# Tung-I/Dual-awareness-Attention-for-Few-shot-Object-Detection

Measured on AMD Instinct MI355X. Metric: query-images/sec (res50, way=2, shot=3, bs=4 per GPU, train-mode forward), higher is better.
Workload: dtype f32 (operands, accumulation, results; multiplies as an exact bf16x3 split, six bf16 MFMA products each)

## Files before the change

### dual-awareness-attention-for-few-shot-object-detection_amd/csrc/igemm.hip

```cpp
#include "common.h"
#include "../../include/dana_hip_debug.h"
#include <stdlib.h>
#include <atomic>

namespace {

typedef float f32x16 __attribute__((ext_vector_type(16)));
typedef unsigned int u32x4 __attribute__((ext_vector_type(4)));

struct IgemmParams {
  const float* A;
  const float* Bw;
  float* C;
  const float* scale;
  const float* shift;
  const float* residual;
  const float* mask;
  long ldm;
  int M, N, K;
  int IH, IW, OH, OW, Cin, KH, KW, stride, pad;
  int M0, IH1, IW1, OH1, OW1, pix1;
  float* C1;
  const float* residual1;
  long ldc1, ldr1;
// ... 6 lines not shown
  int vec_io;
  int vec_ss;
  int tiles_m, tiles_n;
  const float* A2;
  int lda2, IH2, IW2, stride2, K1;
  int IH21, IW21, pix21;
  int bpre;
  const void* Bw2;
  const float* scale2;
  const float* shift2;
  int N2, relu2;
  unsigned a2_bytes;
  int apre, a_rows;
  int res_sample, res_h, res_w, res_oh, res_ow;
  unsigned res_bytes;
  unsigned long long* trace;
};

constexpr int BK = 32;
constexpr int LDS_LD = 36;
constexpr unsigned OOB = 0x80000000u;

__device__ __forceinline__ int xcd_remap(int bid, int nwg) {
  const int q = nwg / 8, r = nwg % 8;
  const int xcd = bid % 8, local = bid / 8;
  return (xcd < r ? xcd * (q + 1) : r * (q + 1) + (xcd - r) * q) + local;
}

__device__ __forceinline__ float4 ldg_b128(__amdgpu_buffer_rsrc_t r, unsigned off) {
  u32x4 v = __builtin_amdgcn_raw_buffer_load_b128(r, (int)off, 0, 0);
// ... 391 lines not shown
#pragma unroll
        for (int r = 0; r < 16; ++r) {
          const int m = m0 + wm * (BM / 2) + i * 32 + (r & 3) + 8 * (r >> 2) + 4 * lh;
          if (m < p.M && ncol[j] < p.N) {
            const bool s1 = m >= p.M0;
            float v = acc[i][j][r] * scv[j] + shv[j];
            if (p.residual) v += s1 ? p.residual1[(long)(m - p.M0) * p.ldr1 + ncol[j]] : p.residual[(long)m * p.ldr + ncol[j]];
            if (p.relu) v = fmaxf(v, 0.f);
            if (p.mask && !(p.mask[(long)m * p.ldm + ncol[j]] > 0.f)) v = 0.f;
            (s1 ? p.C1 + (long)(m - p.M0) * p.ldc1 : Cb + (long)m * p.ldc)[ncol[j]] = v;
          }
        }
  }
}

template <int BM, int BN, int STEM, int BPRE = 0, int FUSE = 0, int ELDS = 0, int RSMP = 0>
__device__ __forceinline__ void igemm_split_body(const IgemmParams& p) {
  static_assert(!RSMP || (!STEM && !FUSE && !ELDS), "sampled residual: register epilogue of the plain conv / GEMM forms");
  constexpr int TM = BM / 64, TN = BN / 64;
  constexpr int RA = BM / 64;
  constexpr int RB = BPRE ? (3 * BN * 2 + 255) / 256 : BN / 64;
  constexpr int CLD = BN + 4;
  extern __shared__ __attribute__((aligned(16))) float smem[];
  unsigned* As = (unsigned*)smem;
  unsigned* Bs = As + 2 * 3 * BM * SLD;

  const int tid = threadIdx.x;
  const int lane = tid & 63, wave = tid >> 6;
  const int wm = wave >> 1, wn = wave & 1;
  const int li = lane & 31, lh = lane >> 5;

  const unsigned long long t_start = p.trace ? __builtin_readcyclecounter() : 0ull;
  const unsigned long long w_start = p.trace ? wall_clock64() : 0ull;
// ... 182 lines not shown
  auto read_frags = [&](int buf, u32x4(&fa)[3][TM], u32x4(&fb)[3][TN]) {
    const unsigned* as = As + buf * 3 * BM * SLD + (wm * (BM / 2) + li) * SLD + rcol;
    const unsigned* bs = Bs + buf * 3 * BN * SLD + (wn * (BN / 2) + li) * SLD + rcol;
#pragma unroll
    for (int pc = 0; pc < 3; ++pc) {
#pragma unroll
      for (int i = 0; i < TM; ++i) fa[pc][i] = *(const u32x4*)(as + (pc * BM + i * 32) * SLD);
#pragma unroll
      for (int j = 0; j < TN; ++j) fb[pc][j] = *(const u32x4*)(bs + (pc * BN + j * 32) * SLD);
    }
  };

  load_tile(ra0, rb0);
  load_tile(ra1, rb1);
  __builtin_amdgcn_sched_barrier(0);
#pragma unroll
  for (int i = 0; i < TM; ++i)
#pragma unroll
    for (int j = 0; j < TN; ++j)
#pragma unroll
      for (int r = 0; r < 16; ++r) acc[i][j][r] = 0.f;
#pragma unroll
  for (int i = 0; i < TM; ++i)
#pragma unroll
    for (int j = 0; j < TN; ++j) asm volatile("" : "+a"(acc[i][j]));
  __builtin_amdgcn_sched_barrier(0);
  store_tile(0, ra0, rb0);
  __syncthreads();
  load_tile(ra0, rb0);
  read_frags(0, fa0, fb0);
  store_tile(1, ra1, rb1);
  __syncthreads();

  auto k_step = [&](int t, const u32x4(&fa)[3][TM], const u32x4(&fb)[3][TN], u32x4(&na)[3][TM], u32x4(&nb)[3][TN],
                    const float4(&cv_a)[RA], const float4(&cv_b)[RB], float4(&ld_a)[RA], float4(&ld_b)[RB]) {
    const int bw_ = t & 1, br_ = bw_ ^ 1;
// ... 422 lines not shown
    }
  }
  if (p.trace && tid == 0) {
    unsigned long long* tr = p.trace + ((long)blockIdx.z * gridDim.x + blockIdx.x) * 8;
    tr[0] = t_start;
    tr[1] = t_loop;
    tr[2] = t_loop_end;
    tr[3] = __builtin_readcyclecounter();
    tr[4] = (unsigned long long)__builtin_amdgcn_s_getreg((31 << 11) | 4) | ((unsigned long long)__builtin_amdgcn_s_getreg((31 << 11) | 20) << 32);
    tr[5] = wall_clock64();
    tr[6] = w_start;
    tr[7] = 0;
  }
}

template <int BM, int BN, int STEM, int BPRE = 0, int FUSE = 0, int ELDS = 0, int RSMP = 0>
__global__ void __launch_bounds__(256, 2) igemm_split_kernel(IgemmParams p) {
  igemm_split_body<BM, BN, STEM, BPRE, FUSE, ELDS, RSMP>(p);
}
template <int STEM, int BPRE, int ELDS, int RSMP = 0>
__global__ void __launch_bounds__(256, 1) __attribute__((amdgpu_num_vgpr(192))) igemm_split_kernel_128(IgemmParams p) {
  igemm_split_body<128, 128, STEM, BPRE, 0, ELDS, RSMP>(p);
}

template <int BN, int NST, int APRE, int DF = 0>
__global__ void __launch_bounds__(256, NST == 2 ? 3 : (NST == 3 ? 2 : 1)) igemm_dma_kernel(IgemmParams p) {
  static_assert(APRE || NST == 2, "fp32 activation rows: two stages");
  static_assert(!DF || (APRE && NST >= 3), "two fragment sets: planes x planes, three or more stages");
  constexpr int BM = 128, TM = 2, TN = BN / 64;
  constexpr int STAGE_B = 3 * (BM + BN) * 32;
  constexpr int NPB = 3 * BN / 32, PB = (NPB + 3) / 4;
  constexpr int NDMA = (APRE ? 3 : 0) + PB;
  constexpr int AHEAD = NST == 2 ? 2 : NST - 1;
  constexpr int RA = BM / 64;
  extern __shared__ __attribute__((aligned(16))) float smem[];
  const int tid = threadIdx.x;
  const int lane = tid & 63, wave = __builtin_amdgcn_readfirstlane(tid >> 6);
// ... 341 lines not shown
  uint2 h, m, l;
  split3(v, h, m, l);
  const int ks = k4 / SBK, kk = k4 - ks * SBK;
  unsigned short* o = out + blockIdx.y * 3 * (long)n * kp + (((long)ks * 3) * n + row) * SBK + kk;
  *(uint2*)o = h;
  *(uint2*)(o + (long)n * SBK) = m;
  *(uint2*)(o + 2 * (long)n * SBK) = l;
}

std::atomic<int>& epilogue_mode_cell() {
  static std::atomic<int> cell(0);
  return cell;
}

std::atomic<int> g_last_form(0);
constexpr int form_code(int family, int bm, int bn, int stem, int bpre, int fuse, int elds, int nst, int apre, int df) {
  return family | (bm / 64) << 4 | (bn / 64) << 6 | stem << 8 | bpre << 9 | fuse << 10 | elds << 11 | nst << 12 | apre << 16 | df << 17;
}

template <int BM, int BN, int STEM>
int launch(const IgemmParams& p0, int batch, hipStream_t s) {
  g_last_form.store(form_code(DANA_IGEMM_FAMILY_F32, BM, BN, STEM, 0, 0, 0, 0, 0, 0), std::memory_order_relaxed);
  IgemmParams p = p0;
  p.tiles_m = (p.M + BM - 1) / BM;
  p.tiles_n = (p.N + BN - 1) / BN;
  size_t lds = (size_t)2 * (BM + BN) * LDS_LD * sizeof(float);
  const size_t lds_c = (size_t)BM * (BN + 4) * sizeof(float);
  if (lds_c > lds) lds = lds_c;
  static DeviceOnce attr;
  attr.once([&] { return hipFuncSetAttribute((const void*)igemm_f32_kernel<BM, BN, STEM>, hipFuncAttributeMaxDynamicSharedMemorySize, (int)lds); });
  dim3 grid(p.tiles_m * p.tiles_n, 1, batch);
  igemm_f32_kernel<BM, BN, STEM><<<grid, 256, lds, s>>>(p);
  return 0;
}

template <int BM, int BN, int STEM = 0, int BPRE = 0, int FUSE = 0, int ELDS = 0, int RSMP = 0>
int launch_split(const IgemmParams& p0, int batch, hipStream_t s) {
  if constexpr (BPRE == 0 && FUSE == 0) {
    if (p0.bpre) return launch_split<BM, BN, STEM, 1, 0, ELDS, RSMP>(p0, batch, s);
  }
  if constexpr (ELDS == 0 && FUSE == 0 && RSMP == 0) {
    if (epilogue_mode_cell().load(std::memory_order_relaxed)) return launch_split<BM, BN, STEM, BPRE, 0, 1>(p0, batch, s);
  }
  g_last_form.store(form_code(BM * BN >= 128 * 128 ? DANA_IGEMM_FAMILY_SPLIT_128 : DANA_IGEMM_FAMILY_SPLIT, BM, BN, STEM, BPRE, FUSE ? 1 : 0,
                              ELDS, 0, 0, 0), std::memory_order_relaxed);
  IgemmParams p = p0;
  p.tiles_m = (p.M + BM - 1) / BM;
  p.tiles_n = (p.N + BN - 1) / BN;
  size_t lds = (size_t)2 * 3 * (BM + BN) * SLD * sizeof(unsigned);
  const size_t lds_c = (size_t)BM * (BN + 4) * sizeof(float);
  if (lds_c > lds && ELDS) lds = lds_c;
  if (FUSE && lds < (size_t)4 * 3 * BM * 16 * 2) lds = (size_t)4 * 3 * BM * 16 * 2;
  if (FUSE == 2 || RSMP) lds += (size_t)BM * 4;
  dim3 grid(p.tiles_m * p.tiles_n, 1, batch);
  static DeviceOnce attr;
  if constexpr (BM * BN >= 128 * 128) {
    attr.once([&] { return hipFuncSetAttribute((const void*)igemm_split_kernel_128<STEM, BPRE, ELDS, RSMP>, hipFuncAttributeMaxDynamicSharedMemorySize,
                                (int)lds); });
    igemm_split_kernel_128<STEM, BPRE, ELDS, RSMP><<<grid, 256, lds, s>>>(p);
  } else {
    attr.once([&] { return hipFuncSetAttribute((const void*)igemm_split_kernel<BM, BN, STEM, BPRE, FUSE, ELDS, RSMP>,
                                hipFuncAttributeMaxDynamicSharedMemorySize, (int)lds); });
    igemm_split_kernel<BM, BN, STEM, BPRE, FUSE, ELDS, RSMP><<<grid, 256, lds, s>>>(p);
  }
  return 0;
}

template <int BN, int NST, int APRE, int DF = 0>
int launch_dma(const IgemmParams& p0, int batch, hipStream_t s) {
  g_last_form.store(form_code(DANA_IGEMM_FAMILY_DMA, 128, BN, 0, 1, 0, 0, NST, APRE, DF), std::memory_order_relaxed);
  IgemmParams p = p0;
  p.tiles_m = (p.M + 127) / 128;
  p.tiles_n = (p.N + BN - 1) / BN;
  const size_t lds = (size_t)NST * 3 * (128 + BN) * 32;
  static DeviceOnce attr;
  attr.once([&] { return hipFuncSetAttribute((const void*)igemm_dma_kernel<BN, NST, APRE, DF>, hipFuncAttributeMaxDynamicSharedMemorySize, (int)lds); });
  dim3 grid(p.tiles_m * p.tiles_n, 1, batch);
  igemm_dma_kernel<BN, NST, APRE, DF><<<grid, 256, lds, s>>>(p);
// ... 31 lines not shown
}
unsigned long long* g_trace = nullptr;

int dispatch_sampled(const IgemmParams& p, int batch, hipStream_t s) {
  const int mode = mfma_mode_cell().load(std::memory_order_relaxed);
  if (!mode || p.apre || p.mask || p.KH * p.KW > 32 || p.M0 != p.M || epilogue_mode_cell().load(std::memory_order_relaxed)) return -1;
  if (p.N <= 64) return -1;
  if (mode == 3) return launch_split<64, 64, 0, 0, 0, 0, 1>(p, batch, s);
  if (mode == 4) return launch_split<128, 128, 0, 0, 0, 0, 1>(p, batch, s);
  if (p.N <= 256 && p.N % 128 != 0 && p.N % 128 <= 32) return launch_split<64, 64, 0, 0, 0, 0, 1>(p, batch, s);
  const long t128 = (long)((p.M + 127) / 128) * ((p.N + 127) / 128) * batch;
  if (t128 < 100) return launch_split<64, 64, 0, 0, 0, 0, 1>(p, batch, s);
  return launch_split<128, 128, 0, 0, 0, 0, 1>(p, batch, s);
}

int dispatch(const IgemmParams& p, int batch, int stem, hipStream_t s) {
  if (p.res_sample) return stem ? -1 : dispatch_sampled(p, batch, s);
  if (stem) {
    const int smode = mfma_mode_cell().load(std::memory_order_relaxed);
    return smode ? launch_split<128, 64, 1>(p, batch, s) : launch<128, 64, 1>(p, batch, s);
  }
  const int mode = mfma_mode_cell().load(std::memory_order_relaxed);
  if (p.apre) {
    const int pp_env = pp_stages_cell().load(std::memory_order_relaxed);
    const long t128 = (long)((p.M + 127) / 128) * ((p.N + 127) / 128) * batch;
    const int stages = pp_env >= 0 ? pp_env : ((t128 < 400 || p.K >= 1024) ? 13 : 2);
    if (p.N <= 64) return stages == 2 ? launch_dma<64, 2, 1>(p, batch, s) : launch_dma<64, 3, 1>(p, batch, s);
    if (stages == 2) return launch_dma<128, 2, 1>(p, batch, s);
    if (stages == 4) return launch_dma<128, 4, 1>(p, batch, s);
    if (stages == 6) return launch_dma<128, 6, 1>(p, batch, s);
    if (stages == 13) return launch_dma<128, 3, 1, 1>(p, batch, s);
// ... 430 lines not shown
                 long batch_a, long batch_b, long batch_c, float alpha, int flags, dana_stream_t stream) {
  DANA_CHECK_ARG(m >= 0 && n >= 0 && k > 0 && batch >= 0, "dana_gemm_nt: bad shape m=%d n=%d k=%d", m, n, k);
  if (m == 0 || n == 0 || batch == 0) return DANA_OK;
  DANA_CHECK_ARG(a && b && c, "dana_gemm_nt: null pointer");
  DANA_CHECK_ARG(k % 4 == 0 && lda % 4 == 0 && ldb % 4 == 0 && batch_a % 4 == 0 && batch_b % 4 == 0,
                 "dana_gemm_nt: k, lda, ldb and batch strides must be multiples of 4 (16-byte rows)");
  const int bpre = (flags & DANA_W_SPLIT3) ? 1 : 0;
  DANA_CHECK_ARG(!bpre || (dana_get_mfma_mode() != 0 && ldb % SBK == 0 && ldb >= k && batch_b % 8 == 0 && n > 8),
                 "dana_gemm_nt: DANA_W_SPLIT3 needs the split kernel, ldb = k rounded up to 16, n > 8");
  const int apre = (flags & DANA_A_SPLIT3) ? 1 : 0;
  DANA_CHECK_ARG(!apre || (bpre && lda % SBK == 0 && lda >= k && batch_a % 8 == 0),
                 "dana_gemm_nt: DANA_A_SPLIT3 needs DANA_W_SPLIT3 too, lda = k rounded up to 16");
  DANA_CHECK_ARG(lda >= k && ldb >= k && ldc >= n, "dana_gemm_nt: leading dimension smaller than the row");
  DANA_CHECK_ARG(((uintptr_t)a & 15) == 0 && ((uintptr_t)b & 15) == 0, "dana_gemm_nt: a/b must be 16-byte aligned");
  DANA_CHECK_ARG(!residual || batch == 1, "dana_gemm_nt: residual only with batch == 1");
  hipStream_t s = (hipStream_t)stream;
  if (n <= 8 && batch == 1 && !residual) {
    gemm_skinny_kernel<8><<<dana_ceil_div(m, 4), 256, 0, s>>>(a, b, c, scale, shift, m, n, k, lda, ldb, ldc, alpha,
                                                              (flags & DANA_EPI_RELU) ? 1 : 0);
    DANA_CHECK_LAUNCH("dana_gemm_nt(skinny)");
    return DANA_OK;
  }
  const long a_bytes = apre ? (long)3 * m * lda * 2 : ((long)(m - 1) * lda + k) * 4;
  const long b_bytes = bpre ? (long)3 * n * ldb * 2 : ((long)(n - 1) * ldb + k) * 4;
  DANA_CHECK_ARG(a_bytes < (long)OOB && b_bytes < (long)OOB, "dana_gemm_nt: operand slice >= 2 GiB; split it");
  IgemmParams p;
  memset(&p, 0, sizeof(p));
  p.A = a;
  p.Bw = b;
  p.C = c;
// ... 13 lines not shown
  p.pad = 0;
  p.lda = (int)lda;
  p.ldb = (int)ldb;
  p.a_bytes = (unsigned)a_bytes;
  p.b_bytes = (unsigned)b_bytes;
  p.ldc = ldc;
  p.ldr = ldr > 0 ? ldr : ldc;
  p.batch_a = apre ? batch_a / 2 : batch_a;
  p.batch_b = bpre ? batch_b / 2 : batch_b;
  p.apre = apre;
  p.a_rows = m;
  p.batch_c = batch_c;
  p.bpre = bpre;
  p.alpha = alpha;
  p.relu = (flags & DANA_EPI_RELU) ? 1 : 0;
  run(p, batch, 0, s);
  DANA_CHECK_LAUNCH("dana_gemm_nt");
  return DANA_OK;
}

}
```

### dual-awareness-attention-for-few-shot-object-detection_amd/csrc/winograd.hip

```cpp
#include "common.h"
#include "../../include/dana_hip.h"

namespace {

typedef unsigned int u32x4 __attribute__((ext_vector_type(4)));
constexpr unsigned OOB = 0x80000000u;

__device__ __forceinline__ float4 f4add(float4 a, float4 b) { return make_float4(a.x + b.x, a.y + b.y, a.z + b.z, a.w + b.w); }
__device__ __forceinline__ float4 f4sub(float4 a, float4 b) { return make_float4(a.x - b.x, a.y - b.y, a.z - b.z, a.w - b.w); }

__global__ void __launch_bounds__(256)
wino_filter_kernel(const float* __restrict__ w, float* __restrict__ U, int cout, int cin) {
  const long i = (long)blockIdx.x * blockDim.x + threadIdx.x;
  if (i >= (long)cout * cin) return;
  const int ci = (int)(i % cin);
  const long co = i / cin;
  float g[3][3];
#pragma unroll
  for (int r = 0; r < 3; ++r)
#pragma unroll
    for (int c = 0; c < 3; ++c) g[r][c] = w[((co * 3 + r) * 3 + c) * cin + ci];
  float t[4][3];
#pragma unroll
  for (int c = 0; c < 3; ++c) {
// ... 572 lines not shown
    wino4_output_kernel<<<dana_ceil_div(p.tiles * N4, 256), 256, 0, s>>>(M, output, scale, shift, mask_act, ldm, h, w, N4,
                                                                        p.th, p.tw, p.tiles, ldc,
                                                                        (flags & DANA_EPI_RELU) ? 1 : 0, 0, 0, res, ldr, res_group);
  DANA_CHECK_LAUNCH("dana_conv3x3_winograd4_nhwc(output transform)");
  return DANA_OK;
}

int dana_conv3x3_winograd4_nhwc_masked(const float* input, const float* u, float* output, const float* scale,
                                       const float* shift, const float* mask_act, int batch, int h, int w, int cin,
                                       int cout, long in_pix_stride, long out_pix_stride, long mask_pix_stride,
                                       int flags, void* workspace, size_t workspace_bytes, dana_stream_t stream) {
  return wino4_impl(input, u, output, scale, shift, mask_act, nullptr, 0, 1, batch, h, w, cin, cout, in_pix_stride,
                    out_pix_stride, mask_pix_stride, flags, workspace, workspace_bytes, stream);
}

int dana_conv3x3_winograd4_nhwc_sub(const float* input, const float* u, float* output, const float* scale,
                                    const float* shift, int batch, int h, int w, int cin, int cout, long in_pix_stride,
                                    long out_pix_stride, int sub, int flags, void* workspace, size_t workspace_bytes,
                                    dana_stream_t stream) {
  return wino4_impl(input, u, output, scale, shift, nullptr, nullptr, 0, 1, batch, h, w, cin, cout, in_pix_stride,
                    out_pix_stride, 0, flags, workspace, workspace_bytes, stream, sub);
}

size_t dana_conv3x3_winograd4_dual_workspace_bytes(int n0, int h0, int w0, int n1, int h1, int w1, int cin, int cout) {
  if (n0 < 0 || n1 < 0 || cin <= 0 || cout <= 0) return 0;
  const long t0 = n0 > 0 ? wino_plan(n0, h0, w0, cin, cout, 4).tiles : 0, t1 = n1 > 0 ? wino_plan(n1, h1, w1, cin, cout, 4).tiles : 0;
  return dana_align_up((size_t)36 * (t0 + t1) * cin * 4, 256) + dana_align_up((size_t)36 * (t0 + t1) * cout * 4, 256);
}

int dana_conv3x3_winograd4_nhwc_dual(const float* input, const float* u, float* out0, float* out1, const float* scale,
// ... 75 lines not shown
```

### dual-awareness-attention-for-few-shot-object-detection_amd/dana.py

```python
import contextlib
import math
import time
from types import SimpleNamespace

import numpy as np
import torch
import torch.nn as nn
import torch.nn.functional as F

from . import ops
from .config import cfg
from . import targets as T
from .cached_inputs import (BankEpisode, ClassSweep, QueryBank, QueryBatch, SupportBank, SupportCache,
                            check_cached_forward, query_batch_size, query_device, read_inputs, resolve_bank_episode,
                            resolve_query_batch, resolve_shot_views)


class Bottleneck(nn.Module):
    expansion = 4

    def __init__(self, inplanes, planes, stride=1, downsample=None):
        super().__init__()
        self.conv1 = nn.Conv2d(inplanes, planes, kernel_size=1, stride=stride, bias=False)
        self.bn1 = nn.BatchNorm2d(planes)
# ... 123 lines not shown
        self.unary_gamma = 0.1
        self.semantic_enhance = semantic_enhance
        self.rpn_reduce_dim = rpn_reduce_dim
        self.rcnn_reduce_dim = rcnn_reduce_dim
        self.pos_encoding = pos_encoding
        self.pool_feat_dim = 1024
        self.rcnn_dim = 64
        self.use_winograd = True
        self.winograd_tile = 4
        self.winograd_min_cin = 128
        self.presplit_weights = True
        self.merge_trunk = False
        self.merge_from = 0
        self.fold_roi_pe = True
        self.fold_roi_attn = True
        self.prefetch_dgrad = "layer4"
        self.rpn_side_role = "wgrad"
        self.nms_inclusive = False
        dim_in = self.pool_feat_dim

        def lin(i, o):
            m = nn.Linear(i, o)
            nn.init.normal_(m.weight, std=0.01)
            nn.init.constant_(m.bias, 0)
            return m

        self.rpn_unary_layer = lin(dim_in, 1)
        self.rcnn_unary_layer = lin(dim_in, 1)
        self.rpn_adapt_q_layer = lin(dim_in, rpn_reduce_dim)
        self.rpn_adapt_k_layer = lin(dim_in, rpn_reduce_dim)
# ... 1050 lines not shown
        return corr, (fh, fw), dict(feat=sfeat, map=(sh_, sw_), kp=kp, unary=unary, s_t=s_t, rpn_done=rpn_done)

    def _rpn_attention(self, f, corr, fh, fw, sup):
        B, Cs, NP, dev, main = f.B, f.Cs, f.NP, f.dev, f.main
        d = self.rpn_reduce_dim
        hw = fh * fw
        L = sup["map"][0] * sup["map"][1]
        K1 = f.shot * L
        kp, unary, s_t = sup["kp"], sup["unary"], sup["s_t"]
        scale, seg_w = self._attn_scale(f)
        _, bq = self._w(self.rpn_adapt_q_layer)
        qb3, qld = self._lin_b(self.rpn_adapt_q_layer)
        qp = ops.gemm_nt(corr, qb3, B * hw, d, 1024, lda=2048, ldb=qld, shift=bq)
        ops.colmean_sub_(qp, B, hw, d)
        f.mark("rpn-level Q projection")
        if sup["rpn_done"] is not None:
            main.wait_event(sup["rpn_done"])
        f.mark("... wait for the support side (trunk + RPN-level K / unary / S^T chain)")
        att = None
        if f.sweep is not None:
            scores = torch.empty((B, hw, Cs * K1), dtype=torch.float32, device=dev)
            ops.gemm_nt(qp, kp, hw, Cs * K1, d, out=scores, ldc=Cs * K1, batch=B, batch_a=hw * d, batch_b=Cs * K1 * d,
                        batch_c=hw * Cs * K1, alpha=1.0 / math.sqrt(d))
            a_p = torch.empty((NP, hw, K1), dtype=torch.float32, device=dev)
            if seg_w is not None:
                ops.attn_softmax_unary_sweep_w(scores, a_p, unary, B, Cs, hw, f.shot, L, K1, K1, K1, self.unary_gamma, seg_w)
            else:
                ops.attn_softmax_unary_sweep(scores, a_p, unary, B, Cs, hw, f.shot, L, K1, K1, K1, self.unary_gamma, scale)
            if f.maps is not None:
                f.maps["rpn_w"] = a_p
# ... 21 lines not shown
        if f.inter is not None:
            f.inter["corr"] = (corr, B, fh, fw)
        if f.ctx is not None:
            f.ctx.update(corr=corr, fh=fh, fw=fw, qp=qp, scores=scores)
        f.mark("rpn-level attention (incl. wait for support stream)")
        return att

    @staticmethod
    def _attn_scale(f):
        if f.maps is None:
            return 1.0 / f.shot, f.seg_w
        if f.seg_w is not None and "slot_w" not in f.maps:
            f.maps["slot_w"] = (f.seg_w > 0).to(torch.float32)
        return 1.0, f.maps.get("slot_w")

    def _rpn_conv_stage(self, f, corr, att, fh, fw):
        if f.sweep is not None:
            return self._rpn_conv_sweep(f.plan, corr, att, f.B, f.Cs, fh, fw, f.product)
        kv = [] if f.ctx is not None else None
        x = self._rpn_conv(f.plan, corr.view(-1)[1024:] if f.product else corr, f.B, fh, fw, in_stride=2048, keep_v=kv)
        if kv:
            f.ctx["rpn_v"] = kv[0]
        return x

    def _roi_support(self, f, sup):
        ctx = f.ctx
        if f.cache is None:
            proposals_start = ops.record_event()
            with ops.on_stream(f.sup_stream):
                f.sup_stream.wait_event(proposals_start)
                sh_, sw_ = sup["map"]
                Ns = f.B * f.way * f.shot
                if f.episode is not None:
# ... 210 lines not shown
```

### dual-awareness-attention-for-few-shot-object-detection_amd/ops.py

```python
import collections
import contextlib
import ctypes
import time as _time

import torch

from ._lib import lib, DanaError

HOST_WAIT = [0.0]

NCHW, NHWC = 0, 1
EPI_RELU, CONV_STEM7, W_SPLIT3, A_SPLIT3 = 1, 2, 256, 512

PROFILE = None
PROF_ROLE = None


def _prof_begin():
    if PROFILE is None:
        return None
    e = torch.cuda.Event(enable_timing=True)
    e.record()
    return e


def _prof_end(e0, tag, flops, nbytes=0.0, executed=None):
    if e0 is not None:
# ... 756 lines not shown
    elif sub != 1:
        lib().call("dana_conv3x3_winograd4_nhwc_sub", _p(x), up, _p(out), _p(scale), _p(shift), batch, h, w, cin, cout,
                   in_stride, out_stride, int(sub), (EPI_RELU if relu else 0) | wfl, _p(ws), ws.numel(), _stream())
    else:
        lib().call("dana_conv3x3_winograd%s_nhwc_masked" % sfx, _p(x), up, _p(out), _p(scale), _p(shift), _p(mask), batch,
                   h, w, cin, cout, in_stride, out_stride, mask_stride, (EPI_RELU if relu else 0) | wfl, _p(ws), ws.numel(),
                   _stream())
    if keep_v is not None and m == 4:
        keep_v.append(ws)
    _prof_end(e0, ("wino3x3 M=%d N=%d K=%d s1", (batch * h * w, cout, 9 * cin)), 2.0 * batch * h * w * cout * 9 * cin,
              4.0 * (m + 2) * (m + 2) * (batch * ((h + m - 1) // m) * ((w + m - 1) // m) * (cin + cout) + cout * cin),
              executed=2.0 * (m + 2) * (m + 2) * batch * ((h + m - 1) // m) * ((w + m - 1) // m) * cin * cout)
    return out, oh, ow


def set_mfma_mode(mode):
    prev = lib().query("dana_get_mfma_mode")
    lib().call("dana_set_mfma_mode", int(mode))
    return prev


def get_mfma_mode():
    return lib().query("dana_get_mfma_mode")


def force_tile(tile):
    lib().call("dana_debug_force_tile", int(tile))


def cumask_stream(cus_per_xcd, n_xcd=8, cus_in_xcd=32):
# ... 28 lines not shown

def get_dma_kernel():
    return lib().query("dana_debug_get_dma_kernel")


def set_pp_stages(v):
    prev = lib().query("dana_debug_get_pp_stages")
    lib().call("dana_debug_set_pp_stages", int(v))
    return prev


def get_pp_stages():
    return lib().query("dana_debug_get_pp_stages")


IgemmForm = collections.namedtuple("IgemmForm", "family bm bn stem bpre fuse elds nst apre df")
_IGEMM_FAMILIES = {0: None, 1: "f32", 2: "split", 3: "split_128", 4: "dma"}


def decode_igemm_form(code):
    return IgemmForm(_IGEMM_FAMILIES[code & 15], (code >> 4 & 3) * 64, (code >> 6 & 3) * 64, code >> 8 & 1, code >> 9 & 1,
                     code >> 10 & 1, code >> 11 & 1, code >> 12 & 15, code >> 16 & 1, code >> 17 & 1)


def last_igemm_form():
    return decode_igemm_form(lib().query("dana_debug_last_igemm_form"))


@contextlib.contextmanager
def igemm_forms(tile=0, dma=-1, pp=-1, epilogue=0):
    prev_dma, prev_pp, prev_epi = get_dma_kernel(), get_pp_stages(), lib().query("dana_get_epilogue_mode")
    try:
        if tile:
            force_tile(tile)
        set_dma_kernel(dma)
        set_pp_stages(pp)
        set_epilogue_mode(epilogue)
# ... 11 lines not shown

def _splitk_slices(m, n, k, batch):
    if batch != 1 or n % 4 or n <= 8 or k < 512 or k % 16:
        return 1
    tiles = ((m + 63) // 64) * ((n + 63) // 64)
    if tiles >= 512:
        return 1
    s = max(1, min(8, round(768.0 / tiles)))
    steps = k // 16
    while s > 1 and (steps % s or k // s < 256):
        s -= 1
    return s


def gemm_nt(a, b, m, n, k, lda=0, ldb=0, out=None, ldc=0, scale=None, shift=None, residual=None, ldr=0, batch=1,
            batch_a=0, batch_b=0, batch_c=0, alpha=1.0, relu=False, k_true=0, force_slices=0):
    bp, wfl = _wf(b)
    if isinstance(a, W3):
        if not wfl or a.n != m or a.k != k or batch != a.batch:
            raise ValueError("gemm_nt: split activation planes need split weights and matching m / k / batch")
        out = torch.empty((batch, m, n) if batch > 1 else (m, n), dtype=torch.float32, device=a.t.device) if out is None else out
        ldc = ldc or n
        e0 = _prof_begin()
        lib().call("dana_gemm_nt", _p(a.t), bp, _p(out), _p(scale), _p(shift), _p(residual), m, n, k, a.kp, b.kp, ldc,
                   ldr, batch, 3 * m * a.kp, 3 * n * b.kp, batch_c or m * n, float(alpha), (EPI_RELU if relu else 0) | wfl | A_SPLIT3,
                   _stream())
        _prof_end(e0, ("gemm M=%d N=%d K=%d b%d", (m, n, k, batch)), 2.0 * batch * m * n * (k_true or k),
                  batch * (6.0 * (m * k + n * k) + 4.0 * m * n * (2 if residual is not None else 1)))
        return out
    _chk(a, "a")
    lda = lda or k
    if wfl:
        if ldb not in (0, k) or batch != 1 or b.n != n or b.k != k:
            raise ValueError("gemm_nt: a split weight is used whole ([n][k] as split)")
        ldb = b.kp
    else:
        ldb = ldb or k
    if out is None:
        out = torch.empty((batch, m, n) if batch > 1 else (m, n), dtype=torch.float32, device=a.device)
        ldc = n
        batch_c = m * n
    e0 = _prof_begin()
    slices = (force_slices or _splitk_slices(m, n, k, batch)) if SPLIT_K else 1
    if wfl and slices > 1 and (k // slices) % 16:
        slices = 1
    if slices > 1:
        kc = k // slices
        part = torch.empty((slices, m, n), dtype=torch.float32, device=a.device)
        lib().call("dana_gemm_nt", _p(a), bp, _p(part), None, None, None, m, n, kc, lda, ldb, n, 0, slices, kc,
                   kc * 3 * n if wfl else kc, m * n, 1.0, wfl, _stream())
        lib().call("dana_splitk_reduce", _p(part), slices, m, n, _p(out), ldc, _p(scale), _p(shift), _p(residual), ldr,
                   float(alpha), EPI_RELU if relu else 0, _stream())
    else:
        lib().call("dana_gemm_nt", _p(a), bp, _p(out), _p(scale), _p(shift), _p(residual), m, n, k, lda, ldb, ldc,
                   ldr, batch, batch_a, batch_b, batch_c, float(alpha), (EPI_RELU if relu else 0) | wfl, _stream())
    _prof_end(e0, ("gemm M=%d N=%d K=%d b%d", (m, n, k, batch)), 2.0 * batch * m * n * (k_true or k),
              4.0 * batch * (m * k + n * k + m * n * (2 if residual is not None else 1)))
    return out


def nchw_to_nhwc(x, cpad=None, out=None, out_stride=0):
    x = _chk(x.contiguous(), "x")
    B, C, H, W = x.shape
    cpad = cpad or C
    if out is None:
        out = torch.empty((B, H, W, cpad), dtype=torch.float32, device=x.device)
    lib().call("dana_nchw_to_nhwc", _p(x), _p(out), B, C, H, W, cpad, out_stride, _stream())
    return out


def nhwc_to_nchw(x, B, C, H, W, in_stride=0):
    _chk(x, "x")
# ... 706 lines not shown
```

### include/dana_hip.h

```cpp
#ifndef DANA_HIP_H
#define DANA_HIP_H
#include <stddef.h>
#include <stdint.h>

#ifdef __cplusplus
extern "C" {
#endif

typedef void* dana_stream_t;

#define DANA_LAYOUT_NCHW 0
#define DANA_LAYOUT_NHWC 1

#define DANA_EPI_RELU 1
#define DANA_CONV_STEM7 2
#define DANA_W_SPLIT3 256
#define DANA_A_SPLIT3 512

const char* dana_last_error(void);
int dana_abi_version(void);

int dana_set_mfma_mode(int mode);
int dana_get_mfma_mode(void);


int dana_roi_align_forward(const float* input, const float* rois, float* output, int batch, int channels,
                           int height, int width, int num_rois, float spatial_scale, int pooled_h,
                           int pooled_w, int sampling_ratio, int layout, long in_pix_stride,
                           long out_pix_stride, float* output2, const float* add2, long out2_pix_stride,
                           dana_stream_t stream);

int dana_roi_align_backward(const float* grad_out, const float* rois, float* grad_in, int batch, int channels,
// ... 128 lines not shown
int dana_conv3x3_winograd_nhwc_masked(const float* input, const float* u, float* output, const float* scale,
                                      const float* shift, const float* mask_act, int batch, int h, int w, int cin,
                                      int cout, long in_pix_stride, long out_pix_stride, long mask_pix_stride,
                                      int flags, void* workspace, size_t workspace_bytes, dana_stream_t stream);

int dana_winograd4_filter_transform(const float* w_packed, float* u, int cout, int cin, dana_stream_t stream);
size_t dana_conv3x3_winograd4_workspace_bytes(int batch, int h, int w, int cin, int cout);
int dana_conv3x3_winograd4_nhwc_masked(const float* input, const float* u, float* output, const float* scale,
                                       const float* shift, const float* mask_act, int batch, int h, int w, int cin,
                                       int cout, long in_pix_stride, long out_pix_stride, long mask_pix_stride,
                                       int flags, void* workspace, size_t workspace_bytes, dana_stream_t stream);
int dana_conv3x3_winograd4_nhwc_sub(const float* input, const float* u, float* output, const float* scale,
                                    const float* shift, int batch, int h, int w, int cin, int cout, long in_pix_stride,
                                    long out_pix_stride, int sub, int flags, void* workspace, size_t workspace_bytes,
                                    dana_stream_t stream);
int dana_conv3x3_winograd_nhwc_grouped_res(const float* input, const float* u, float* output, const float* scale,
                                           const float* shift, const float* residual, int batch, int h, int w, int cin,
                                           int cout, long in_pix_stride, long out_pix_stride, long res_pix_stride,
                                           int res_group, int tile, int flags, void* workspace, size_t workspace_bytes,
                                           dana_stream_t stream);
size_t dana_conv3x3_winograd4_dual_workspace_bytes(int n0, int h0, int w0, int n1, int h1, int w1, int cin, int cout);
int dana_conv3x3_winograd4_nhwc_dual(const float* input, const float* u, float* out0, float* out1, const float* scale,
                                     const float* shift, int n0, int h0, int w0, int n1, int h1, int w1, int cin,
                                     int cout, long in_pix_stride, long out0_pix_stride, long out1_pix_stride, int flags,
                                     void* workspace, size_t workspace_bytes, dana_stream_t stream);
int dana_conv3x3_winograd4_nhwc_dual_masked(const float* input, const float* u, float* out0, float* out1,
                                            const float* scale, const float* shift, const float* mask0,
                                            const float* mask1, int n0, int h0, int w0, int n1, int h1, int w1, int cin,
                                            int cout, long in_pix_stride, long out0_pix_stride, long out1_pix_stride,
                                            long mask0_pix_stride, long mask1_pix_stride, int flags, void* workspace,
// ... 296 lines not shown
```

Baseline: 731.7.

## Start RPN 3x3 conv on first half of channels before waiting on support side

Adds a channel-range-partitioned Winograd F(4x4,3x3) conv whose GEMM can seed its accumulators from the existing output, so a conv can be split into two K-halves. The first half of the RPN conv (channels 0-1024 of the query-only correlation input) is launched before the main stream waits on the support-side event, and the second half plus the output transform runs afterwards. This moves work off the critical path behind the cross-stream wait. In exchange the seeded GEMM rereads and rewrites the M workspace, paying one extra input-transform launch and extra memory traffic.

```diff
diff --git a/dual-awareness-attention-for-few-shot-object-detection_amd/csrc/igemm.hip b/dual-awareness-attention-for-few-shot-object-detection_amd/csrc/igemm.hip
--- a/dual-awareness-attention-for-few-shot-object-detection_amd/csrc/igemm.hip
+++ b/dual-awareness-attention-for-few-shot-object-detection_amd/csrc/igemm.hip
@@ -44,6 +44,7 @@
   int apre, a_rows;
   int res_sample, res_h, res_w, res_oh, res_ow;
   unsigned res_bytes;
+  int seed;
   unsigned long long* trace;
 };
 
@@ -465,9 +466,10 @@
   }
 }
 
-template <int BM, int BN, int STEM, int BPRE = 0, int FUSE = 0, int ELDS = 0, int RSMP = 0>
+template <int BM, int BN, int STEM, int BPRE = 0, int FUSE = 0, int ELDS = 0, int RSMP = 0, int SEED = 0>
 __device__ __forceinline__ void igemm_split_body(const IgemmParams& p) {
   static_assert(!RSMP || (!STEM && !FUSE && !ELDS), "sampled residual: register epilogue of the plain conv / GEMM forms");
+  static_assert(!SEED || (!STEM && !FUSE && !ELDS && !RSMP), "seeded accumulators: register epilogue of the plain GEMM forms");
   constexpr int TM = BM / 64, TN = BN / 64;
   constexpr int RA = BM / 64;
   constexpr int RB = BPRE ? (3 * BN * 2 + 255) / 256 : BN / 64;
@@ -680,12 +682,31 @@
   load_tile(ra0, rb0);
   load_tile(ra1, rb1);
   __builtin_amdgcn_sched_barrier(0);
-#pragma unroll
-  for (int i = 0; i < TM; ++i)
-#pragma unroll
-    for (int j = 0; j < TN; ++j)
-#pragma unroll
-      for (int r = 0; r < 16; ++r) acc[i][j][r] = 0.f;
+  if constexpr (SEED) {
+    const int rows_valid = (p.M - m0) < BM ? (p.M - m0) : BM;
+    const int ldc4 = (int)p.ldc * 4;
+    const __amdgpu_buffer_rsrc_t rc_seed =
+        __builtin_amdgcn_make_buffer_rsrc((void*)(Cb + (long)m0 * p.ldc), 0, rows_valid * ldc4, 0x00020000);
+    const int lrow = wm * (BM / 2) + 4 * lh;
+#pragma unroll
+    for (int j = 0; j < TN; ++j) {
+      const int ncol = n0 + wn * (BN / 2) + j * 32 + li;
+      const unsigned vo = ncol < p.N ? (unsigned)(lrow * ldc4 + ncol * 4) : OOB;
+#pragma unroll
+      for (int i = 0; i < TM; ++i)
+#pragma unroll
+        for (int r = 0; r < 16; ++r)
+          acc[i][j][r] = __builtin_bit_cast(
+              float, __builtin_amdgcn_raw_buffer_load_b32(rc_seed, (int)(vo + (unsigned)((i * 32 + (r & 3) + 8 * (r >> 2)) * ldc4)), 0, 0));
+    }
+  } else {
+#pragma unroll
+    for (int i = 0; i < TM; ++i)
+#pragma unroll
+      for (int j = 0; j < TN; ++j)
+#pragma unroll
+        for (int r = 0; r < 16; ++r) acc[i][j][r] = 0.f;
+  }
 #pragma unroll
   for (int i = 0; i < TM; ++i)
 #pragma unroll
@@ -1138,13 +1159,13 @@
   }
 }
 
-template <int BM, int BN, int STEM, int BPRE = 0, int FUSE = 0, int ELDS = 0, int RSMP = 0>
+template <int BM, int BN, int STEM, int BPRE = 0, int FUSE = 0, int ELDS = 0, int RSMP = 0, int SEED = 0>
 __global__ void __launch_bounds__(256, 2) igemm_split_kernel(IgemmParams p) {
-  igemm_split_body<BM, BN, STEM, BPRE, FUSE, ELDS, RSMP>(p);
-}
-template <int STEM, int BPRE, int ELDS, int RSMP = 0>
+  igemm_split_body<BM, BN, STEM, BPRE, FUSE, ELDS, RSMP, SEED>(p);
+}
+template <int STEM, int BPRE, int ELDS, int RSMP = 0, int SEED = 0>
 __global__ void __launch_bounds__(256, 1) __attribute__((amdgpu_num_vgpr(192))) igemm_split_kernel_128(IgemmParams p) {
-  igemm_split_body<128, 128, STEM, BPRE, 0, ELDS, RSMP>(p);
+  igemm_split_body<128, 128, STEM, BPRE, 0, ELDS, RSMP, SEED>(p);
 }
 
 template <int BN, int NST, int APRE, int DF = 0>
@@ -1516,8 +1537,9 @@
 }
 
 std::atomic<int> g_last_form(0);
-constexpr int form_code(int family, int bm, int bn, int stem, int bpre, int fuse, int elds, int nst, int apre, int df) {
-  return family | (bm / 64) << 4 | (bn / 64) << 6 | stem << 8 | bpre << 9 | fuse << 10 | elds << 11 | nst << 12 | apre << 16 | df << 17;
+constexpr int form_code(int family, int bm, int bn, int stem, int bpre, int fuse, int elds, int nst, int apre, int df, int seed = 0) {
+  return family | (bm / 64) << 4 | (bn / 64) << 6 | stem << 8 | bpre << 9 | fuse << 10 | elds << 11 | nst << 12 | apre << 16 | df << 17 |
+         seed << 18;
 }
 
 template <int BM, int BN, int STEM>
@@ -1536,16 +1558,16 @@
   return 0;
 }
 
-template <int BM, int BN, int STEM = 0, int BPRE = 0, int FUSE = 0, int ELDS = 0, int RSMP = 0>
+template <int BM, int BN, int STEM = 0, int BPRE = 0, int FUSE = 0, int ELDS = 0, int RSMP = 0, int SEED = 0>
 int launch_split(const IgemmParams& p0, int batch, hipStream_t s) {
   if constexpr (BPRE == 0 && FUSE == 0) {
-    if (p0.bpre) return launch_split<BM, BN, STEM, 1, 0, ELDS, RSMP>(p0, batch, s);
-  }
-  if constexpr (ELDS == 0 && FUSE == 0 && RSMP == 0) {
+    if (p0.bpre) return launch_split<BM, BN, STEM, 1, 0, ELDS, RSMP, SEED>(p0, batch, s);
+  }
+  if constexpr (ELDS == 0 && FUSE == 0 && RSMP == 0 && SEED == 0) {
     if (epilogue_mode_cell().load(std::memory_order_relaxed)) return launch_split<BM, BN, STEM, BPRE, 0, 1>(p0, batch, s);
   }
   g_last_form.store(form_code(BM * BN >= 128 * 128 ? DANA_IGEMM_FAMILY_SPLIT_128 : DANA_IGEMM_FAMILY_SPLIT, BM, BN, STEM, BPRE, FUSE ? 1 : 0,
-                              ELDS, 0, 0, 0), std::memory_order_relaxed);
+                              ELDS, 0, 0, 0, SEED), std::memory_order_relaxed);
   IgemmParams p = p0;
   p.tiles_m = (p.M + BM - 1) / BM;
   p.tiles_n = (p.N + BN - 1) / BN;
@@ -1557,13 +1579,13 @@
   dim3 grid(p.tiles_m * p.tiles_n, 1, batch);
   static DeviceOnce attr;
   if constexpr (BM * BN >= 128 * 128) {
-    attr.once([&] { return hipFuncSetAttribute((const void*)igemm_split_kernel_128<STEM, BPRE, ELDS, RSMP>, hipFuncAttributeMaxDynamicSharedMemorySize,
+    attr.once([&] { return hipFuncSetAttribute((const void*)igemm_split_kernel_128<STEM, BPRE, ELDS, RSMP, SEED>, hipFuncAttributeMaxDynamicSharedMemorySize,
                                 (int)lds); });
-    igemm_split_kernel_128<STEM, BPRE, ELDS, RSMP><<<grid, 256, lds, s>>>(p);
+    igemm_split_kernel_128<STEM, BPRE, ELDS, RSMP, SEED><<<grid, 256, lds, s>>>(p);
   } else {
-    attr.once([&] { return hipFuncSetAttribute((const void*)igemm_split_kernel<BM, BN, STEM, BPRE, FUSE, ELDS, RSMP>,
+    attr.once([&] { return hipFuncSetAttribute((const void*)igemm_split_kernel<BM, BN, STEM, BPRE, FUSE, ELDS, RSMP, SEED>,
                                 hipFuncAttributeMaxDynamicSharedMemorySize, (int)lds); });
-    igemm_split_kernel<BM, BN, STEM, BPRE, FUSE, ELDS, RSMP><<<grid, 256, lds, s>>>(p);
+    igemm_split_kernel<BM, BN, STEM, BPRE, FUSE, ELDS, RSMP, SEED><<<grid, 256, lds, s>>>(p);
   }
   return 0;
 }
@@ -1625,7 +1647,27 @@
   return launch_split<128, 128, 0, 0, 0, 0, 1>(p, batch, s);
 }
 
+int dispatch_seeded(const IgemmParams& p, int batch, hipStream_t s) {
+  const int mode = mfma_mode_cell().load(std::memory_order_relaxed);
+  if (!mode || p.apre || p.mask || p.res_sample || p.A2 || p.KH * p.KW != 1 || p.M0 != p.M ||
+      epilogue_mode_cell().load(std::memory_order_relaxed))
+    return -1;
+  if (p.N <= 64 || mode == 2 || mode == 5) return -1;
+  const long t128 = (long)((p.M + 127) / 128) * ((p.N + 127) / 128) * batch;
+  if (mode == 1 && p.bpre) {
+    const int dm_env = dma_kernel_cell().load(std::memory_order_relaxed);
+    const int dm = dm_env >= 0 ? dm_env : 1;
+    if (dm == 2 || (dm == 1 && t128 >= 600 && p.K <= 192)) return -1;
+  }
+  if (mode == 3) return launch_split<64, 64, 0, 0, 0, 0, 0, 1>(p, batch, s);
+  if (mode == 4) return launch_split<128, 128, 0, 0, 0, 0, 0, 1>(p, batch, s);
+  if (p.N <= 256 && p.N % 128 != 0 && p.N % 128 <= 32) return launch_split<64, 64, 0, 0, 0, 0, 0, 1>(p, batch, s);
+  if (t128 < 100) return launch_split<64, 64, 0, 0, 0, 0, 0, 1>(p, batch, s);
+  return launch_split<128, 128, 0, 0, 0, 0, 0, 1>(p, batch, s);
+}
+
 int dispatch(const IgemmParams& p, int batch, int stem, hipStream_t s) {
+  if (p.seed) return stem ? -1 : dispatch_seeded(p, batch, s);
   if (p.res_sample) return stem ? -1 : dispatch_sampled(p, batch, s);
   if (stem) {
     const int smode = mfma_mode_cell().load(std::memory_order_relaxed);
@@ -2086,6 +2128,10 @@
   DANA_CHECK_ARG(lda >= k && ldb >= k && ldc >= n, "dana_gemm_nt: leading dimension smaller than the row");
   DANA_CHECK_ARG(((uintptr_t)a & 15) == 0 && ((uintptr_t)b & 15) == 0, "dana_gemm_nt: a/b must be 16-byte aligned");
   DANA_CHECK_ARG(!residual || batch == 1, "dana_gemm_nt: residual only with batch == 1");
+  const int seed = (flags & DANA_GEMM_SEED) ? 1 : 0;
+  DANA_CHECK_ARG(!seed || (alpha == 1.f && !scale && !shift && !residual && !(flags & DANA_EPI_RELU) && !apre && n > 64),
+                 "dana_gemm_nt: DANA_GEMM_SEED continues a plain accumulation: alpha = 1, no scale / shift / residual / ReLU, "
+                 "fp32 activation rows, n > 64");
   hipStream_t s = (hipStream_t)stream;
   if (n <= 8 && batch == 1 && !residual) {
     gemm_skinny_kernel<8><<<dana_ceil_div(m, 4), 256, 0, s>>>(a, b, c, scale, shift, m, n, k, lda, ldb, ldc, alpha,
@@ -2129,7 +2175,10 @@
   p.bpre = bpre;
   p.alpha = alpha;
   p.relu = (flags & DANA_EPI_RELU) ? 1 : 0;
-  run(p, batch, 0, s);
+  p.seed = seed;
+  const int rc = run(p, batch, 0, s);
+  DANA_CHECK_ARG(!seed || rc == 0, "dana_gemm_nt: DANA_GEMM_SEED needs the split kernel's register epilogue at a 64 x 64 or "
+                                   "128 x 128 tile (dana_set_mfma_mode(1), no LDS epilogue, not the DMA kernel); nothing was launched");
   DANA_CHECK_LAUNCH("dana_gemm_nt");
   return DANA_OK;
 }
diff --git a/dual-awareness-attention-for-few-shot-object-detection_amd/csrc/winograd.hip b/dual-awareness-attention-for-few-shot-object-detection_amd/csrc/winograd.hip
--- a/dual-awareness-attention-for-few-shot-object-detection_amd/csrc/winograd.hip
+++ b/dual-awareness-attention-for-few-shot-object-detection_amd/csrc/winograd.hip
@@ -610,6 +610,61 @@
                     out_pix_stride, mask_pix_stride, flags, workspace, workspace_bytes, stream);
 }
 
+size_t dana_conv3x3_winograd4_part_workspace_bytes(int batch, int h, int w, int cin, int cout) {
+  return dana_conv3x3_winograd4_workspace_bytes(batch, h, w, cin, cout);
+}
+
+int dana_conv3x3_winograd4_nhwc_part(const float* input, const float* u, float* output, const float* scale,
+                                     const float* shift, int batch, int h, int w, int cin, int cout, int k0, int k1,
+                                     long in_pix_stride, long out_pix_stride, int flags, void* workspace,
+                                     size_t workspace_bytes, dana_stream_t stream) {
+  const char* who = "dana_conv3x3_winograd4_nhwc_part";
+  DANA_CHECK_ARG(batch >= 0 && h > 0 && w > 0 && cin > 0 && cout > 0 && cin % 4 == 0 && cout % 4 == 0, "%s: bad shape", who);
+  DANA_CHECK_ARG(k0 >= 0 && k0 < k1 && k1 <= cin && k0 % 16 == 0 && (k1 % 16 == 0 || k1 == cin),
+                 "%s: the channel range [%d, %d) must lie in [0, %d) and be cut at multiples of 16", who, k0, k1, cin);
+  if (batch == 0) return DANA_OK;
+  DANA_CHECK_ARG(input && u && output, "%s: null pointer", who);
+  const long lda = in_pix_stride > 0 ? in_pix_stride : cin;
+  const long ldc = out_pix_stride > 0 ? out_pix_stride : cout;
+  DANA_CHECK_ARG(lda >= cin && lda % 4 == 0 && ldc % 4 == 0 && ((uintptr_t)input & 15) == 0 && ((uintptr_t)output & 15) == 0,
+                 "%s: strides / pointers must be 16-byte aligned", who);
+  const WinoPlan p = wino_plan(batch, h, w, cin, cout, 4);
+  if (!workspace || workspace_bytes < p.total) {
+    dana_set_error("%s: workspace %zu < %zu", who, workspace_bytes, p.total);
+    return DANA_ERR_WORKSPACE;
+  }
+  const bool first = k0 == 0, last = k1 == cin;
+  if (cout <= 64) {
+    if (!last) return DANA_OK;
+    return wino4_impl(input, u, output, scale, shift, nullptr, nullptr, 0, 1, batch, h, w, cin, cout, in_pix_stride,
+                      out_pix_stride, 0, flags, workspace, workspace_bytes, stream);
+  }
+  const int kc = k1 - k0;
+  const long in_bytes = (long)batch * h * w * lda * 4 - (long)k0 * 4;
+  DANA_CHECK_ARG(in_bytes < (long)OOB, "%s: input span >= 2 GiB; split the batch", who);
+  hipStream_t s = (hipStream_t)stream;
+  float* V = (float*)workspace;
+  float* M = (float*)((char*)workspace + p.v_bytes);
+  const int C4 = kc / 4, N4 = cout / 4;
+  DANA_CHECK_ARG(p.tiles * (long)(cin / 4 > N4 ? cin / 4 : N4) < (1L << 31), "%s: too many tiles x channels", who);
+  wino4_input_kernel<<<dana_ceil_div(p.tiles * C4, 256), 256, 0, s>>>(input + k0, V, h, w, C4, p.th, p.tw, p.tiles, (int)lda,
+                                                                     (unsigned)in_bytes);
+  DANA_CHECK_LAUNCH("dana_conv3x3_winograd4_nhwc_part(input transform)");
+  const bool w3 = (flags & DANA_W_SPLIT3) != 0;
+  const long kp = (cin + 15) / 16 * 16, kcp = (kc + 15) / 16 * 16;
+  const float* ub = w3 ? (const float*)((const unsigned short*)u + (long)k0 * 3 * cout) : u + k0;
+  int rc = dana_gemm_nt(V, ub, M, nullptr, nullptr, nullptr, (int)p.tiles, cout, kc, kc, w3 ? kcp : cin, cout, 0, 36,
+                        p.tiles * kc, w3 ? 3 * cout * kp : (long)cout * cin, p.tiles * cout, 1.f,
+                        (w3 ? DANA_W_SPLIT3 : 0) | (first ? 0 : DANA_GEMM_SEED), stream);
+  if (rc) return rc;
+  if (!last) return DANA_OK;
+  wino4_output_kernel<<<dana_ceil_div(p.tiles * N4, 256), 256, 0, s>>>(M, output, scale, shift, nullptr, cout, h, w, N4, p.th,
+                                                                      p.tw, p.tiles, ldc, (flags & DANA_EPI_RELU) ? 1 : 0, 0,
+                                                                      0, nullptr, cout, 1);
+  DANA_CHECK_LAUNCH("dana_conv3x3_winograd4_nhwc_part(output transform)");
+  return DANA_OK;
+}
+
 int dana_conv3x3_winograd4_nhwc_sub(const float* input, const float* u, float* output, const float* scale,
                                     const float* shift, int batch, int h, int w, int cin, int cout, long in_pix_stride,
                                     long out_pix_stride, int sub, int flags, void* workspace, size_t workspace_bytes,
diff --git a/dual-awareness-attention-for-few-shot-object-detection_amd/dana.py b/dual-awareness-attention-for-few-shot-object-detection_amd/dana.py
--- a/dual-awareness-attention-for-few-shot-object-detection_amd/dana.py
+++ b/dual-awareness-attention-for-few-shot-object-detection_amd/dana.py
@@ -161,6 +161,7 @@
         self.merge_from = 0
         self.fold_roi_pe = True
         self.fold_roi_attn = True
+        self.early_rpn_half = True
         self.prefetch_dgrad = "layer4"
         self.rpn_side_role = "wgrad"
         self.nms_inclusive = False
@@ -1241,6 +1242,11 @@
         qp = ops.gemm_nt(corr, qb3, B * hw, d, 1024, lda=2048, ldb=qld, shift=bq)
         ops.colmean_sub_(qp, B, hw, d)
         f.mark("rpn-level Q projection")
+        f.rpn_ws = None
+        if self._early_rpn_half(f, sup):
+            f.rpn_ws = ops.conv3x3_winograd_part_workspace(B, fh, fw, 2048, 512, dev)
+            ops.conv3x3_winograd_part(corr, B, fh, fw, 2048, f.plan["rpn_conv_b3"] or f.plan["rpn_conv_u"], 512, 0, 1024,
+                                      f.rpn_ws, in_stride=2048)
         if sup["rpn_done"] is not None:
             main.wait_event(sup["rpn_done"])
         f.mark("... wait for the support side (trunk + RPN-level K / unary / S^T chain)")
@@ -1292,9 +1298,18 @@
             f.maps["slot_w"] = (f.seg_w > 0).to(torch.float32)
         return 1.0, f.maps.get("slot_w")
 
+    def _early_rpn_half(self, f, sup):
+        return (getattr(self, "early_rpn_half", True) and f.ctx is None and sup["rpn_done"] is not None
+                and ops.get_mfma_mode() == 1 and ops.get_epilogue_mode() == 0
+                and f.sup_stream != f.main and f.sweep is None and f.maps is None and not f.product
+                and f.plan["rpn_conv_u"] is not None and self.winograd_tile == 4 and self.RCNN_rpn.din == 2048)
+
     def _rpn_conv_stage(self, f, corr, att, fh, fw):
         if f.sweep is not None:
             return self._rpn_conv_sweep(f.plan, corr, att, f.B, f.Cs, fh, fw, f.product)
+        if getattr(f, "rpn_ws", None) is not None:
+            return ops.conv3x3_winograd_part(corr, f.B, fh, fw, 2048, f.plan["rpn_conv_b3"] or f.plan["rpn_conv_u"], 512,
+                                             1024, 2048, f.rpn_ws, shift=f.plan["rpn_conv_b"], relu=True, in_stride=2048)
         kv = [] if f.ctx is not None else None
         x = self._rpn_conv(f.plan, corr.view(-1)[1024:] if f.product else corr, f.B, fh, fw, in_stride=2048, keep_v=kv)
         if kv:
diff --git a/dual-awareness-attention-for-few-shot-object-detection_amd/ops.py b/dual-awareness-attention-for-few-shot-object-detection_amd/ops.py
--- a/dual-awareness-attention-for-few-shot-object-detection_amd/ops.py
+++ b/dual-awareness-attention-for-few-shot-object-detection_amd/ops.py
@@ -10,7 +10,7 @@
 HOST_WAIT = [0.0]
 
 NCHW, NHWC = 0, 1
-EPI_RELU, CONV_STEM7, W_SPLIT3, A_SPLIT3 = 1, 2, 256, 512
+EPI_RELU, CONV_STEM7, W_SPLIT3, A_SPLIT3, GEMM_SEED = 1, 2, 256, 512, 1024
 
 PROFILE = None
 PROF_ROLE = None
@@ -797,6 +797,29 @@
     return out, oh, ow
 
 
+def conv3x3_winograd_part_workspace(batch, h, w, cin, cout, device):
+    return _ws(lib().query("dana_conv3x3_winograd4_part_workspace_bytes", batch, h, w, cin, cout), device)
+
+
+def conv3x3_winograd_part(x, batch, h, w, cin, u, cout, k0, k1, ws, scale=None, shift=None, relu=False, in_stride=0, out=None,
+                          out_stride=0):
+    _chk(x, "x")
+    up, wfl = _wf(u)
+    if (u.batch if isinstance(u, W3) else u.size(0)) != 36:
+        raise ValueError("conv3x3_winograd_part: F(4x4,3x3) filters only")
+    if k1 == cin and out is None:
+        out = torch.empty((batch * h * w, cout), dtype=torch.float32, device=x.device)
+        out_stride = cout
+    e0 = _prof_begin()
+    lib().call("dana_conv3x3_winograd4_nhwc_part", _p(x), up, _p(out if out is not None else ws), _p(scale), _p(shift), batch,
+               h, w, cin, cout, k0, k1, in_stride, out_stride, (EPI_RELU if relu else 0) | wfl, _p(ws), ws.numel(), _stream())
+    tiles = batch * ((h + 3) // 4) * ((w + 3) // 4)
+    _prof_end(e0, ("wino3x3 part M=%d N=%d K=%d s1", (batch * h * w, cout, 9 * (k1 - k0))),
+              2.0 * batch * h * w * cout * 9 * (k1 - k0), 4.0 * 36 * (tiles * (k1 - k0 + cout * (1 if k0 == 0 else 2)) + cout * (k1 - k0)),
+              executed=2.0 * 36 * tiles * (k1 - k0) * cout)
+    return out if k1 == cin else None
+
+
 def set_mfma_mode(mode):
     prev = lib().query("dana_get_mfma_mode")
     lib().call("dana_set_mfma_mode", int(mode))
@@ -855,13 +878,13 @@
     return lib().query("dana_debug_get_pp_stages")
 
 
-IgemmForm = collections.namedtuple("IgemmForm", "family bm bn stem bpre fuse elds nst apre df")
+IgemmForm = collections.namedtuple("IgemmForm", "family bm bn stem bpre fuse elds nst apre df seed", defaults=(0,))
 _IGEMM_FAMILIES = {0: None, 1: "f32", 2: "split", 3: "split_128", 4: "dma"}
 
 
 def decode_igemm_form(code):
     return IgemmForm(_IGEMM_FAMILIES[code & 15], (code >> 4 & 3) * 64, (code >> 6 & 3) * 64, code >> 8 & 1, code >> 9 & 1,
-                     code >> 10 & 1, code >> 11 & 1, code >> 12 & 15, code >> 16 & 1, code >> 17 & 1)
+                     code >> 10 & 1, code >> 11 & 1, code >> 12 & 15, code >> 16 & 1, code >> 17 & 1, code >> 18 & 1)
 
 
 def last_igemm_form():
@@ -903,8 +926,12 @@
 
 
 def gemm_nt(a, b, m, n, k, lda=0, ldb=0, out=None, ldc=0, scale=None, shift=None, residual=None, ldr=0, batch=1,
-            batch_a=0, batch_b=0, batch_c=0, alpha=1.0, relu=False, k_true=0, force_slices=0):
+            batch_a=0, batch_b=0, batch_c=0, alpha=1.0, relu=False, k_true=0, force_slices=0, seed=False, b_step0=None):
     bp, wfl = _wf(b)
+    if seed and (out is None or alpha != 1.0 or relu or scale is not None or shift is not None or residual is not None
+                 or isinstance(a, W3) or force_slices > 1):
+        raise ValueError("gemm_nt: a seeded launch continues a plain accumulation in `out`: alpha 1, no epilogue term, "
+                         "fp32 activation rows, no split-K")
     if isinstance(a, W3):
         if not wfl or a.n != m or a.k != k or batch != a.batch:
             raise ValueError("gemm_nt: split activation planes need split weights and matching m / k / batch")
@@ -919,7 +946,11 @@
         return out
     _chk(a, "a")
     lda = lda or k
-    if wfl:
+    if wfl and b_step0 is not None:
+        if batch != b.batch or b.n != n or k % 16 or b_step0 < 0 or b_step0 * 16 + k > b.kp:
+            raise ValueError("gemm_nt: a K range of a split weight is whole K-steps of its [batch][n][k] planes")
+        bp, ldb, batch_b = bp + b_step0 * 3 * n * 16 * 2, k, 3 * n * b.kp
+    elif wfl:
         if ldb not in (0, k) or batch != 1 or b.n != n or b.k != k:
             raise ValueError("gemm_nt: a split weight is used whole ([n][k] as split)")
         ldb = b.kp
@@ -930,7 +961,7 @@
         ldc = n
         batch_c = m * n
     e0 = _prof_begin()
-    slices = (force_slices or _splitk_slices(m, n, k, batch)) if SPLIT_K else 1
+    slices = (force_slices or _splitk_slices(m, n, k, batch)) if SPLIT_K and not seed and b_step0 is None else 1
     if wfl and slices > 1 and (k // slices) % 16:
         slices = 1
     if slices > 1:
@@ -942,9 +973,10 @@
                    float(alpha), EPI_RELU if relu else 0, _stream())
     else:
         lib().call("dana_gemm_nt", _p(a), bp, _p(out), _p(scale), _p(shift), _p(residual), m, n, k, lda, ldb, ldc,
-                   ldr, batch, batch_a, batch_b, batch_c, float(alpha), (EPI_RELU if relu else 0) | wfl, _stream())
+                   ldr, batch, batch_a, batch_b, batch_c, float(alpha),
+                   (EPI_RELU if relu else 0) | wfl | (GEMM_SEED if seed else 0), _stream())
     _prof_end(e0, ("gemm M=%d N=%d K=%d b%d", (m, n, k, batch)), 2.0 * batch * m * n * (k_true or k),
-              4.0 * batch * (m * k + n * k + m * n * (2 if residual is not None else 1)))
+              4.0 * batch * (m * k + n * k + m * n * (2 if residual is not None or seed else 1)))
     return out
 
 
diff --git a/include/dana_hip.h b/include/dana_hip.h
--- a/include/dana_hip.h
+++ b/include/dana_hip.h
@@ -16,6 +16,7 @@
 #define DANA_CONV_STEM7 2
 #define DANA_W_SPLIT3 256
 #define DANA_A_SPLIT3 512
+#define DANA_GEMM_SEED 1024
 
 const char* dana_last_error(void);
 int dana_abi_version(void);
@@ -174,6 +175,11 @@
                                     const float* shift, int batch, int h, int w, int cin, int cout, long in_pix_stride,
                                     long out_pix_stride, int sub, int flags, void* workspace, size_t workspace_bytes,
                                     dana_stream_t stream);
+size_t dana_conv3x3_winograd4_part_workspace_bytes(int batch, int h, int w, int cin, int cout);
+int dana_conv3x3_winograd4_nhwc_part(const float* input, const float* u, float* output, const float* scale,
+                                     const float* shift, int batch, int h, int w, int cin, int cout, int k0, int k1,
+                                     long in_pix_stride, long out_pix_stride, int flags, void* workspace,
+                                     size_t workspace_bytes, dana_stream_t stream);
 int dana_conv3x3_winograd_nhwc_grouped_res(const float* input, const float* u, float* output, const float* scale,
                                            const float* shift, const float* residual, int batch, int h, int w, int cin,
                                            int cout, long in_pix_stride, long out_pix_stride, long res_pix_stride,
```

Result: no change. 733.3 (median of 3 runs) (+0.2%).
